# uc-vision/smart-tree

Hardware: AMD Instinct MI355X
Metric: points/sec end-to-end (voxelize->sparse-UNet->skeleton), 1M-pt tree (higher is better)
Workload: dtype f32

## Files before the change

smart_tree_amd/csrc/knn.hip:

```cpp
#include "st_common.h"
#include "st_grid.h"

#define KNN_BLOCK 256

#define KNN_MEAN_MULT 0.45f

__global__ void k_grid_init(StGrid* g) {
    if (threadIdx.x == 0 && blockIdx.x == 0) {
        for (int a = 0; a < 3; a++) { g->lo_ord[a] = 0xffffffffu; g->hi_ord[a] = 0u; }
        g->rmax_ord = 0u;
        g->bound_sum_fix = 0ull;
        g->bound_cnt = 0ull;
        g->r = 0.0f;
    }
    if (blockIdx.x == 0 && threadIdx.x < ST_MAX_SEG) { g->seg_rmax_ord[threadIdx.x] = 0u; g->seg_r[threadIdx.x] = 0.0f; }
}

__device__ __forceinline__ unsigned grid_wave_min(unsigned v) { for (int d = 32; d > 0; d >>= 1) { const unsigned o = __shfl_xor(v, d); v = o < v ? o : v; } return v; }
__device__ __forceinline__ unsigned grid_wave_max(unsigned v) { for (int d = 32; d > 0; d >>= 1) { const unsigned o = __shfl_xor(v, d); v = o > v ? o : v; } return v; }

__global__ void __launch_bounds__(KNN_BLOCK) k_bound_max(const float* bound, int64_t n, StGrid* g, const int* seg_off, const uint8_t* valid) {
    __shared__ unsigned m;
    __shared__ unsigned long long sum, cnt;
    if (threadIdx.x == 0) { m = 0u; sum = 0ull; cnt = 0ull; }
    __syncthreads();
    const int seg = blockIdx.y;
    const int64_t i0 = seg_off ? seg_off[seg] : 0, i1 = seg_off ? seg_off[seg + 1] : n;
    unsigned mine = 0u;
    unsigned long long fix = 0ull;
    unsigned long long seen = 0ull;
    for (int64_t i = i0 + (int64_t)blockIdx.x * blockDim.x + threadIdx.x; i < i1; i += (int64_t)gridDim.x * blockDim.x) {
        if (valid && !valid[i]) continue;
        const float b = bound[i];
        if (b != b) continue;
        const unsigned o = st_f2ord(b);
        if (o > mine) mine = o;
        fix += (unsigned long long)(fminf(fmaxf(b, 0.0f), 128.0f) * 65536.0f);
        seen++;
    }
    mine = grid_wave_max(mine);
    for (int d = 32; d > 0; d >>= 1) { fix += __shfl_xor(fix, d); seen += __shfl_xor(seen, d); }
    if ((threadIdx.x & 63) == 0) { if (mine) atomicMax(&m, mine); atomicAdd(&sum, fix); atomicAdd(&cnt, seen); }
    __syncthreads();
    if (threadIdx.x == 0) {
        if (m) { atomicMax(&g->rmax_ord, m); atomicMax(&g->seg_rmax_ord[seg], m); }
        if (sum) atomicAdd(&g->bound_sum_fix, sum);
        if (cnt) atomicAdd(&g->bound_cnt, cnt);
    }
}

__global__ void __launch_bounds__(KNN_BLOCK) k_grid_bbox(const float* pts, int64_t n, StGrid* g, const uint8_t* valid) {
    __shared__ unsigned lo[3], hi[3];
    if (threadIdx.x < 3) { lo[threadIdx.x] = 0xffffffffu; hi[threadIdx.x] = 0u; }
    __syncthreads();
    unsigned l[3] = {0xffffffffu, 0xffffffffu, 0xffffffffu}, h[3] = {0u, 0u, 0u};
    const int64_t total = 3 * n, step = (int64_t)gridDim.x * blockDim.x;
    const int64_t e0 = (int64_t)blockIdx.x * blockDim.x + threadIdx.x;
    const int step3 = (int)(step % 3);
    int a = (int)(e0 % 3);
    for (int64_t e = e0; e < total; e += step, a = (a + step3) % 3) {
        const float pv = pts[e];
        if (valid && !valid[e / 3]) continue;
        if (!(fabsf(pv) <= 3.0e38f)) continue;
        const unsigned o = st_f2ord(pv);
#pragma unroll
        for (int k = 0; k < 3; k++)
            if (a == k) { l[k] = o < l[k] ? o : l[k]; h[k] = o > h[k] ? o : h[k]; }
    }
#pragma unroll
    for (int a = 0; a < 3; a++) { l[a] = grid_wave_min(l[a]); h[a] = grid_wave_max(h[a]); }
    if ((threadIdx.x & 63) == 0)
        for (int a = 0; a < 3; a++) { atomicMin(&lo[a], l[a]); atomicMax(&hi[a], h[a]); }
    __syncthreads();
    if (threadIdx.x < 3 && lo[threadIdx.x] <= hi[threadIdx.x]) {
        atomicMin(&g->lo_ord[threadIdx.x], lo[threadIdx.x]);
        atomicMax(&g->hi_ord[threadIdx.x], hi[threadIdx.x]);
    }
}

__global__ void k_grid_dims(StGrid* g, float cell, int64_t max_cells, float r, int nseg, float mean_mult, int64_t n_bound) {
    if (threadIdx.x != 0 || blockIdx.x != 0) return;
    float lo[3], hi[3];
    for (int a = 0; a < 3; a++) { lo[a] = st_ord2f(g->lo_ord[a]); hi[a] = st_ord2f(g->hi_ord[a]); g->lo[a] = lo[a]; }
    for (int s = 0; s < nseg; s++) g->seg_r[s] = r < 0.0f ? st_ord2f(g->seg_rmax_ord[s]) : r;
    if (r < 0.0f) r = st_ord2f(g->rmax_ord);
    g->r = r;
    if (cell < 0.0f) {
        cell = r / -cell;
        if (mean_mult > 0.0f && n_bound > 0 && g->bound_cnt > 0ull) {
            const float mean = (float)((double)g->bound_sum_fix / 65536.0 / (double)g->bound_cnt);
            if (mean > 0.0f) cell = fminf(cell, mean_mult * mean);
        }
        cell = fmaxf(cell, 1e-4f);
    }
    if (!(cell > 0.0f) || !(cell <= 3.0e38f)) cell = 1.0f;
    g->nseg = nseg;
    for (int a = 0; a < 3; a++)
        if (!(hi[a] >= lo[a])) { lo[a] = hi[a] = 0.0f; g->lo[a] = 0.0f; }
    for (int it = 0;; it++) {
        double total = (double)nseg;
        for (int a = 0; a < 3; a++) {
            float ext = (hi[a] - lo[a]) / cell;
            int d = ext < 2.0e9f ? (int)floorf(ext) + 1 : 0x7fffffff;
            if (d < 1 || it >= 300) d = 1;
            g->dim[a] = d;
            total *= (double)d;
        }
        if (total <= (double)max_cells) break;
        cell *= 2.0f;
    }
    g->seg_dim0 = g->dim[0];
    g->dim[0] = g->seg_dim0 * nseg;
    g->cell = cell;
    g->ncell = (int64_t)g->dim[0] * g->dim[1] * g->dim[2];
}

__global__ void k_grid_ncell1(const StGrid* g, int64_t* out) { *out = g->ncell + 1; }

__global__ void __launch_bounds__(KNN_BLOCK) k_grid_count(const float* pts, int64_t n, const StGrid* g, uint32_t* counts,
                                                          const int* seg_off, int nseg, uint32_t* pt_cell, uint32_t* pt_rank,
                                                          const uint8_t* valid) {
    for (int64_t i = (int64_t)blockIdx.x * blockDim.x + threadIdx.x; i < n; i += (int64_t)gridDim.x * blockDim.x) {
        if (valid && !valid[i]) { pt_cell[i] = 0xffffffffu; continue; }
        const float x = pts[3 * i], y = pts[3 * i + 1], z = pts[3 * i + 2];
        const bool finite = fabsf(x) <= 3.0e38f && fabsf(y) <= 3.0e38f && fabsf(z) <= 3.0e38f;
        const int64_t c = st_grid_cell(g, finite ? x : g->lo[0], finite ? y : g->lo[1], finite ? z : g->lo[2], st_seg_find(seg_off, nseg, i));
        pt_cell[i] = (uint32_t)c;
        pt_rank[i] = atomicAdd(&counts[c], 1u);
    }
}

__global__ void __launch_bounds__(KNN_BLOCK) k_grid_fill(const float* pts, int64_t n, const uint32_t* cell_start,
                                                         const uint32_t* pt_cell, const uint32_t* pt_rank, float4* recs) {
    for (int64_t i = (int64_t)blockIdx.x * blockDim.x + threadIdx.x; i < n; i += (int64_t)gridDim.x * blockDim.x) {
        if (pt_cell[i] == 0xffffffffu) continue;
        const uint32_t pos = cell_start[pt_cell[i]] + pt_rank[i];
        recs[pos] = make_float4(pts[3 * i], pts[3 * i + 1], pts[3 * i + 2], __uint_as_float((unsigned)i));
    }
}

int64_t st_grid_ws_bytes(int64_t n, int64_t max_cells) {
    StArena a(nullptr, 0);
    a.take<uint32_t>(n);
    a.take<uint32_t>(n);
    a.take<int64_t>(1);
    a.take<char>(st_scan_ws_bytes(max_cells + 1));
    return a.used;
}

int st_grid_build(const float* pts, int64_t n, float cell, int64_t max_cells, StGrid* g, uint32_t* cell_start, float4* recs,
                  void* ws, int64_t ws_bytes, hipStream_t stream, float r, const float* bound, int64_t n_bound,
                  const int* seg_off, int nseg, const int* bound_seg_off, float mean_mult, const uint8_t* valid) {
    if (nseg < 1 || nseg > ST_MAX_SEG) { st_set_error("grid: 1 <= clouds per batch <= %d (got %d)", ST_MAX_SEG, nseg); return ST_ERR_INVALID; }
    if (!seg_off) nseg = 1;
    StArena a(ws, ws_bytes);
    uint32_t* pt_cell = a.take<uint32_t>(n);
    uint32_t* pt_rank = a.take<uint32_t>(n);
    int64_t* ncell1_dev = a.take<int64_t>(1);
    int64_t scan_bytes = st_scan_ws_bytes(max_cells + 1);
    char* scan_ws = a.take<char>(scan_bytes);
    if (!pt_cell || !pt_rank || !ncell1_dev || !scan_ws) {
        st_set_error("grid: workspace too small (%lld < %lld)", (long long)ws_bytes, (long long)a.used);
        return ST_ERR_WORKSPACE;
    }
    unsigned gb = (unsigned)st_min64(st_div_up(n > 0 ? n : 1, KNN_BLOCK), 4096);
    hipLaunchKernelGGL(k_grid_init, dim3(1), dim3(64), 0, stream, g);
    static_assert(ST_MAX_SEG <= 64, "k_grid_init clears the per-cloud radii with one wavefront");
    hipLaunchKernelGGL(k_grid_bbox, dim3((unsigned)st_min64(st_div_up(3 * (n > 0 ? n : 1), (int64_t)KNN_BLOCK * 8), 512)), dim3(KNN_BLOCK), 0, stream, pts, n, g, valid);
    const int64_t ncell = st_min64(max_cells, 128 * n + 65536);
    if (r < 0.0f && bound && n_bound > 0)
        hipLaunchKernelGGL(k_bound_max, dim3((unsigned)st_min64(st_div_up(n_bound, (int64_t)KNN_BLOCK * nseg * 8), 512 / nseg + 1), (unsigned)nseg),
                           dim3(KNN_BLOCK), 0, stream, bound, n_bound, g, nseg > 1 ? (bound_seg_off ? bound_seg_off : seg_off) : (const int*)nullptr,
                           valid);
    hipLaunchKernelGGL(k_grid_dims, dim3(1), dim3(64), 0, stream, g, cell, ncell, r, nseg, mean_mult,
                       (r < 0.0f && bound) ? n_bound : (int64_t)0);
    if (getenv("ST_GRID_DEBUG")) {
        StGrid h;
        (void)hipMemcpyAsync(&h, g, sizeof(StGrid), hipMemcpyDeviceToHost, stream);
        st_stream_wait(stream);
        fprintf(stderr, "grid: n=%lld cell=%g ncell=%lld of %lld dims=%d,%d,%d\n", (long long)n, h.cell, (long long)h.ncell,
                (long long)ncell, h.dim[0], h.dim[1], h.dim[2]);
    }
    hipLaunchKernelGGL(k_grid_ncell1, dim3(1), dim3(1), 0, stream, (const StGrid*)g, ncell1_dev);
    st_fill_u32_dev(cell_start, ncell + 1, ncell1_dev, 0u, stream);
    hipLaunchKernelGGL(k_grid_count, dim3(gb), dim3(KNN_BLOCK), 0, stream, pts, n, (const StGrid*)g, cell_start, seg_off, nseg,
                       pt_cell, pt_rank, valid);
    ST_TRY(st_exclusive_scan_u32(cell_start, cell_start, ncell + 1, nullptr, scan_ws, scan_bytes, stream, ncell1_dev));
    hipLaunchKernelGGL(k_grid_fill, dim3(gb), dim3(KNN_BLOCK), 0, stream, pts, n, (const uint32_t*)cell_start,
                       (const uint32_t*)pt_cell, (const uint32_t*)pt_rank, recs);
    ST_CHECK_LAUNCH();
    return ST_OK;
}


#define KNN_WAVES (KNN_BLOCK / 64)
#define KNN_MASK_WORDS 64
#define KNN_CAP 128

__device__ __forceinline__ uint32_t knn_wave_scan(uint32_t v, int lane) {
    for (int d = 1; d < 64; d <<= 1) { const uint32_t o = __shfl_up(v, (unsigned)d); if (lane >= d) v += o; }
    return v;
}

__device__ __forceinline__ float knn_d2_max(float bound, bool strict) {
    if (!(bound >= 0.0f)) return -1.0f;
    if (bound == __uint_as_float(0x7f800000u)) return strict ? __uint_as_float(0x7f7fffffu) : bound;
    auto pass = [&](float x) { const float s = sqrtf(x); return strict ? s < bound : s <= bound; };
    unsigned b = __float_as_uint(bound * bound);
    if (b > 0x7f7fffffu) b = 0x7f7fffffu;
    while (!pass(__uint_as_float(b))) { if (b == 0u) return -1.0f; b--; }
    while (b < 0x7f7fffffu && pass(__uint_as_float(b + 1u))) b++;
    return __uint_as_float(b);
}

struct __attribute__((aligned(16))) KnnPair { unsigned long long x, y; };

template <int NCH, class F>
__device__ __forceinline__ void knn_rank(const unsigned long long* keys, int n, int lane, F emit) {
    unsigned long long mine[NCH];
    int rank[NCH];
#pragma unroll
    for (int c = 0; c < NCH; c++) {
        const int j = c * 64 + lane;
        mine[c] = j < n ? keys[j] : ~0ull;
        rank[c] = 0;
    }
    int t = 0;
    for (; t + 4 <= n; t += 4) {
        const KnnPair a = *reinterpret_cast<const KnnPair*>(keys + t), b = *reinterpret_cast<const KnnPair*>(keys + t + 2);
#pragma unroll
        for (int c = 0; c < NCH; c++)
            rank[c] += (a.x < mine[c] ? 1 : 0) + (a.y < mine[c] ? 1 : 0) + (b.x < mine[c] ? 1 : 0) + (b.y < mine[c] ? 1 : 0);
    }
    for (; t < n; t++) {
        const unsigned long long kt = keys[t];
#pragma unroll
        for (int c = 0; c < NCH; c++) rank[c] += kt < mine[c] ? 1 : 0;
    }
    __builtin_amdgcn_wave_barrier();
#pragma unroll
    for (int c = 0; c < NCH; c++)
        if (c * 64 + lane < n) emit(mine[c], rank[c]);
}

template <int K>
__device__ __forceinline__ int knn_cut(unsigned long long* keys, int n, int lane) {
    __builtin_amdgcn_wave_barrier();
    auto put = [&](unsigned long long key, int rank) { if (rank < K) keys[rank] = key; };
    if (n <= 64) knn_rank<1>(keys, n, lane, put); else knn_rank<KNN_CAP / 64>(keys, n, lane, put);
    __builtin_amdgcn_wave_barrier();
    return n < K ? n : K;
}

template <int K, bool COUNT = false>
__global__ void __launch_bounds__(KNN_BLOCK, 8) k_knn(const float* __restrict__ src, int64_t n1, const StGrid* __restrict__ g,
                                                   const uint32_t* __restrict__ cell_start, const float4* __restrict__ recs,
                                                   float r, const float* __restrict__ bound, int mode,
                                                   int64_t* __restrict__ idx_out, float* __restrict__ dist_out,
                                                   const int* __restrict__ seg_off, int nseg, int cell_order,
                                                   const uint8_t* __restrict__ valid = nullptr) {
    __shared__ uint32_t s_roff[KNN_WAVES][65], s_rfirst[KNN_WAVES][64];
    __shared__ unsigned long long s_rmask[KNN_WAVES][KNN_MASK_WORDS];
    __shared__ __attribute__((aligned(16))) unsigned long long s_keys[KNN_WAVES][KNN_CAP];
    const int lane = threadIdx.x & 63, wave = threadIdx.x >> 6;
    int64_t i = (int64_t)blockIdx.x * KNN_WAVES + wave;
    if (i >= n1) return;
    if (valid && (cell_order ? i >= (int64_t)cell_start[g->ncell] : !valid[i])) return;
    float px, py, pz;
    if (cell_order) {
        const float4 me = recs[i];
        px = me.x; py = me.y; pz = me.z;
        i = (int64_t)__float_as_uint(me.w);
    } else {
        px = src[3 * i]; py = src[3 * i + 1]; pz = src[3 * i + 2];
    }
    uint32_t* roff = s_roff[wave];
    uint32_t* rfirst = s_rfirst[wave];
    unsigned long long* rmask = s_rmask[wave];
    unsigned long long* keys = s_keys[wave];
    const int seg = st_seg_find(seg_off, nseg, i);
    if (r < 0.0f) r = g->seg_r[seg];
    const float r2 = r * r;
    float reach_r = r;
    float d2_max = __uint_as_float(0x7f800000u);
    if (mode != 0) {
        const float bnd = bound[i];
        if (bnd < reach_r) reach_r = bnd;
        d2_max = knn_d2_max(bnd, mode == 2);
    }
    const float cell = g->cell;
    const float reach_f = reach_r > 0.0f ? ceilf(reach_r / cell) : 0.0f;
    int reach = reach_f < 1.0e6f ? (int)reach_f : 1000000;
    if (reach < 1) reach = 1;
    const bool q_finite = fabsf(px) <= 3.0e38f && fabsf(py) <= 3.0e38f && fabsf(pz) <= 3.0e38f;
    if (!q_finite) { px = g->lo[0]; py = g->lo[1]; pz = g->lo[2]; reach = 0; d2_max = -1.0f; }
    const int cx = (int)floorf((px - g->lo[0]) / cell), cy = (int)floorf((py - g->lo[1]) / cell), cz = (int)floorf((pz - g->lo[2]) / cell);
    const int xoff = seg * g->seg_dim0;
    const int x0 = st_max(cx - reach, 0), x1 = st_min(cx + reach, g->seg_dim0 - 1);
    const int y0 = st_max(cy - reach, 0), y1 = st_min(cy + reach, g->dim[1] - 1);
    const int z0 = st_max(cz - reach, 0), z1 = st_min(cz + reach, g->dim[2] - 1);
    const float rs = reach_r * 1.0001f + 1e-7f, rs2 = rs * rs;
    const int ny = y1 - y0 + 1, nrows = (x1 >= x0 && ny > 0 && z1 >= z0) ? (x1 - x0 + 1) * ny : 0;
    int nkeys = 0;
    unsigned long long thr = ~0ull;
    for (int rbase = 0; rbase < nrows && !(COUNT && nkeys >= K); rbase += 64) {
        const int rowi = rbase + lane;
        uint32_t first = 0, cnt = 0;
        if (rowi < nrows) {
            const int x = x0 + rowi / ny, y = y0 + rowi % ny;
            const float cx0 = g->lo[0] + (float)x * cell, ex = px < cx0 ? cx0 - px : (px > cx0 + cell ? px - (cx0 + cell) : 0.0f);
            const float cy0 = g->lo[1] + (float)y * cell, ey = py < cy0 ? cy0 - py : (py > cy0 + cell ? py - (cy0 + cell) : 0.0f);
            const float dxy2 = ex * ex + ey * ey;
            if (!(dxy2 > rs2)) {
                const float rz = sqrtf(rs2 - dxy2);
                const int za = (int)fmaxf(floorf((pz - rz - g->lo[2]) / cell) - 1.0f, (float)z0),
                          zb = (int)fminf(floorf((pz + rz - g->lo[2]) / cell) + 1.0f, (float)z1);
                if (za <= zb) {
                    const int64_t row = ((int64_t)(xoff + x) * g->dim[1] + y) * g->dim[2];
                    first = cell_start[row + za];
                    cnt = cell_start[row + zb + 1] - first;
                }
            }
        }
        const uint32_t incl = knn_wave_scan(cnt, lane);
        const int total = (int)__shfl(incl, 63);
        const unsigned long long nonempty = __ballot(cnt != 0u);
        const int nr = __popcll(nonempty);
        const int slot = __popcll(nonempty & ((1ull << lane) - 1ull));
        const bool marks = total <= 64 * KNN_MASK_WORDS;
        __builtin_amdgcn_wave_barrier();
        if (marks)
            for (int w = lane; w < (total + 63) / 64; w += 64) rmask[w] = 0ull;
        if (cnt != 0u) { roff[slot] = incl - cnt; rfirst[slot] = first; }
        if (lane == 63) roff[nr] = incl;
        __builtin_amdgcn_wave_barrier();
        if (marks && cnt != 0u) atomicOr(&rmask[(incl - cnt) >> 6], 1ull << ((incl - cnt) & 63u));
        __builtin_amdgcn_wave_barrier();
        int rows_before = 0;
        for (int cb = 0; cb < total && !(COUNT && nkeys >= K); cb += 64) {
            const int t = cb + lane;
            bool ok = false;
            unsigned long long key = 0ull;
            const unsigned long long starts = marks ? rmask[cb >> 6] : 0ull;
            if (t < total) {
                int lo;
                if (marks) {
                    lo = rows_before + __popcll(starts & (~0ull >> (63 - lane))) - 1;
                } else {
                    lo = 0;
                    int hi = nr;
                    while (hi - lo > 1) { const int mid = (lo + hi) >> 1; if (roff[mid] <= (uint32_t)t) lo = mid; else hi = mid; }
                }
                const float4 q = recs[rfirst[lo] + ((uint32_t)t - roff[lo])];
                const float dx = px - q.x, dy = py - q.y, dz = pz - q.z;
                float d2 = dx * dx;
                float tt = dy * dy;
                d2 = d2 + tt;
                tt = dz * dz;
                d2 = d2 + tt;
                ok = d2 < r2 && d2 <= d2_max;
                key = ((unsigned long long)__float_as_uint(d2) << 32) | (unsigned long long)__float_as_uint(q.w);
                if (!COUNT) ok = ok && key < thr;
            }
            const unsigned long long bal = __ballot(ok);
            if (!COUNT && ok) keys[nkeys + __popcll(bal & ((1ull << lane) - 1ull))] = key;
            nkeys += __popcll(bal);
            if (!COUNT && nkeys > KNN_CAP - 64) {
                nkeys = knn_cut<K>(keys, nkeys, lane);
                if (nkeys == K) thr = keys[K - 1];
            }
            rows_before += __popcll(starts);
        }
    }
    if (COUNT) {
        if (lane == 0) reinterpret_cast<uint8_t*>(idx_out)[i] = nkeys >= K ? 1 : 0;
        return;
    }
    __builtin_amdgcn_wave_barrier();
    {
        auto put = [&](unsigned long long key, int rank) {
            if (rank < K) {
                idx_out[i * K + rank] = (int64_t)(unsigned)(key & 0xffffffffull);
                dist_out[i * K + rank] = sqrtf(__uint_as_float((unsigned)(key >> 32)));
            }
        };
        if (nkeys <= 64) knn_rank<1>(keys, nkeys, lane, put); else knn_rank<KNN_CAP / 64>(keys, nkeys, lane, put);
        const int found = nkeys < K ? nkeys : K;
        if (lane >= found && lane < K) {
            idx_out[i * K + lane] = (int64_t)-1;
            dist_out[i * K + lane] = __uint_as_float(0x7fc00000u);
        }
    }
}

#define KNN_MAX_CELLS (1ll << 24)
static inline int64_t knn_max_cells(int nseg) { return KNN_MAX_CELLS * (nseg < 1 ? 1 : (nseg > 32 ? 32 : nseg)); }

static inline int64_t knn_cells(int64_t n2, int nseg) { return st_min64(knn_max_cells(nseg), 128 * (n2 > 0 ? n2 : 1) + 65536); }

static void knn_layout(StArena& a, int64_t n2, int nseg, StGrid** g, uint32_t** cell_start, float4** recs, char** sub, int64_t* sub_bytes) {
    *g = a.take<StGrid>(1);
    *cell_start = a.take<uint32_t>(knn_cells(n2, nseg) + 1);
    *recs = a.take<float4>(n2);
    *sub_bytes = st_grid_ws_bytes(n2, knn_cells(n2, nseg));
    *sub = a.take<char>(*sub_bytes);
}

extern "C" int64_t st_knn_workspace_bytes_seg(int64_t n_dst, int nseg) {
    StArena a(nullptr, 0);
    StGrid* g; uint32_t* cs; float4* recs; char* sub; int64_t sb;
    knn_layout(a, n_dst, nseg, &g, &cs, &recs, &sub, &sb);
    return a.used;
}
extern "C" int64_t st_knn_workspace_bytes(int64_t n_dst) { return st_knn_workspace_bytes_seg(n_dst, 1); }

extern "C" int st_knn_radius_seg(const float* src, int64_t n1, const float* dst, int64_t n2, int K, float r, const float* bound,
                                 int bound_mode, float cell_hint, int64_t* idx, float* dist, const int32_t* src_seg_off,
                                 const int32_t* dst_seg_off, int nseg, void* ws, int64_t ws_bytes, void* stream_,
                                 float cell_mean_mult) {
    hipStream_t stream = (hipStream_t)stream_;
    ST_REQUIRE(K == 1 || K == 8 || K == 16 || K == 32 || K == 64, "knn: K must be 1, 8, 16, 32 or 64 (got %d)", K);
    static_assert(KNN_CAP >= 128, "a cut keeps K <= 64 keys and the next chunk adds up to 64");
    ST_REQUIRE(bound_mode == 0 || bound != nullptr, "knn: bound_mode needs a bound array");
    ST_REQUIRE(r >= 0.0f || bound != nullptr, "knn: r < 0 (radius = max(bound)) needs a bound array");
    ST_REQUIRE(cell_hint >= 0.0f || r < 0.0f, "knn: a relative cell size (cell_hint < 0) goes with r < 0");
    ST_REQUIRE(n2 < (1ll << 31), "knn: too many points");
    ST_REQUIRE(nseg >= 1 && nseg <= ST_MAX_SEG, "knn: 1 <= clouds per batch <= %d", ST_MAX_SEG);
    ST_REQUIRE(nseg == 1 || (src_seg_off && dst_seg_off), "knn: a batch needs the cloud offsets of src and dst");
    if (nseg == 1) { src_seg_off = nullptr; dst_seg_off = nullptr; }
    if (n1 <= 0) return ST_OK;
    StArena a(ws, ws_bytes);
    StGrid* g; uint32_t* cell_start; float4* recs; char* sub; int64_t sub_bytes;
    knn_layout(a, n2, nseg, &g, &cell_start, &recs, &sub, &sub_bytes);
    if (!a.ok() || !sub) {
        st_set_error("knn: workspace too small (%lld < %lld)", (long long)ws_bytes, (long long)a.used);
        return ST_ERR_WORKSPACE;
    }
    const float cell_arg = cell_hint != 0.0f ? cell_hint : (r >= 0.0f ? r : -1.0f);
    ST_TRY(st_grid_build(dst, n2, cell_arg, knn_cells(n2, nseg), g, cell_start, recs, sub, sub_bytes, stream, r, bound, n1,
                         dst_seg_off, nseg, src_seg_off, cell_hint < 0.0f ? (cell_mean_mult >= 0.0f ? cell_mean_mult : KNN_MEAN_MULT) : 0.0f, nullptr));
    dim3 grid((unsigned)st_div_up(n1, KNN_WAVES)), block(KNN_BLOCK);
    const int cell_order = src == dst && n1 == n2 ? 1 : 0;
    if (K == 1)
        hipLaunchKernelGGL((k_knn<1>), grid, block, 0, stream, src, n1, (const StGrid*)g, (const uint32_t*)cell_start,
                           (const float4*)recs, r, bound, bound_mode, idx, dist, src_seg_off, nseg, cell_order);
    else if (K == 8)
        hipLaunchKernelGGL((k_knn<8>), grid, block, 0, stream, src, n1, (const StGrid*)g, (const uint32_t*)cell_start,
                           (const float4*)recs, r, bound, bound_mode, idx, dist, src_seg_off, nseg, cell_order);
    else if (K == 16)
        hipLaunchKernelGGL((k_knn<16>), grid, block, 0, stream, src, n1, (const StGrid*)g, (const uint32_t*)cell_start,
                           (const float4*)recs, r, bound, bound_mode, idx, dist, src_seg_off, nseg, cell_order);
    else if (K == 32)
        hipLaunchKernelGGL((k_knn<32>), grid, block, 0, stream, src, n1, (const StGrid*)g, (const uint32_t*)cell_start,
                           (const float4*)recs, r, bound, bound_mode, idx, dist, src_seg_off, nseg, cell_order);
    else
        hipLaunchKernelGGL((k_knn<64>), grid, block, 0, stream, src, n1, (const StGrid*)g, (const uint32_t*)cell_start,
                           (const float4*)recs, r, bound, bound_mode, idx, dist, src_seg_off, nseg, cell_order);
    ST_CHECK_LAUNCH();
    return ST_OK;
}

extern "C" int st_radius_count_seg(const float* src, int64_t n1, const float* dst, int64_t n2, int K, float r, const float* bound,
                                   int bound_mode, float cell_hint, uint8_t* mask, const int32_t* src_seg_off,
                                   const int32_t* dst_seg_off, int nseg, void* ws, int64_t ws_bytes, void* stream_,
                                   float cell_mean_mult, const uint8_t* valid) {
    hipStream_t stream = (hipStream_t)stream_;
    ST_REQUIRE(valid == nullptr || (src == dst && n1 == n2), "radius_count: a validity mask needs src == dst");
    ST_REQUIRE(K == 8, "radius_count: K must be 8 (outlier_removal's nb_points; got %d)", K);
    ST_REQUIRE(bound_mode == 0 || bound != nullptr, "radius_count: bound_mode needs a bound array");
    ST_REQUIRE(r >= 0.0f || bound != nullptr, "radius_count: r < 0 (radius = max(bound)) needs a bound array");
    ST_REQUIRE(cell_hint >= 0.0f || r < 0.0f, "radius_count: a relative cell size (cell_hint < 0) goes with r < 0");
    ST_REQUIRE(n2 < (1ll << 31), "radius_count: too many points");
    ST_REQUIRE(nseg >= 1 && nseg <= ST_MAX_SEG, "radius_count: 1 <= clouds per batch <= %d", ST_MAX_SEG);
    ST_REQUIRE(nseg == 1 || (src_seg_off && dst_seg_off), "radius_count: a batch needs the cloud offsets of src and dst");
    if (nseg == 1) { src_seg_off = nullptr; dst_seg_off = nullptr; }
    if (n1 <= 0) return ST_OK;
    StArena a(ws, ws_bytes);
    StGrid* g; uint32_t* cell_start; float4* recs; char* sub; int64_t sub_bytes;
    knn_layout(a, n2, nseg, &g, &cell_start, &recs, &sub, &sub_bytes);
    if (!a.ok() || !sub) {
        st_set_error("radius_count: workspace too small (%lld < %lld)", (long long)ws_bytes, (long long)a.used);
        return ST_ERR_WORKSPACE;
    }
    const float cell_arg = cell_hint != 0.0f ? cell_hint : (r >= 0.0f ? r : -1.0f);
    ST_TRY(st_grid_build(dst, n2, cell_arg, knn_cells(n2, nseg), g, cell_start, recs, sub, sub_bytes, stream, r, bound, n1,
                         dst_seg_off, nseg, src_seg_off, cell_hint < 0.0f ? (cell_mean_mult >= 0.0f ? cell_mean_mult : KNN_MEAN_MULT) : 0.0f, valid));
    if (valid) (void)hipMemsetAsync(mask, 0, (size_t)n1, stream);
    hipLaunchKernelGGL((k_knn<8, true>), dim3((unsigned)st_div_up(n1, KNN_WAVES)), dim3(KNN_BLOCK), 0, stream, src, n1,
                       (const StGrid*)g, (const uint32_t*)cell_start, (const float4*)recs, r, bound, bound_mode,
                       reinterpret_cast<int64_t*>(mask), (float*)nullptr, src_seg_off, nseg, src == dst && n1 == n2 ? 1 : 0, valid);
    ST_CHECK_LAUNCH();
    return ST_OK;
}

extern "C" int st_knn_radius(const float* src, int64_t n1, const float* dst, int64_t n2, int K, float r, const float* bound,
                             int bound_mode, float cell_hint, int64_t* idx, float* dist, void* ws, int64_t ws_bytes,
                             void* stream_) {
    return st_knn_radius_seg(src, n1, dst, n2, K, r, bound, bound_mode, cell_hint, idx, dist, nullptr, nullptr, 1, ws, ws_bytes,
                             stream_, -1.0f);
}
```

smart_tree_amd/csrc/prims.hip:

```cpp
#include <cstdarg>

#include "st_common.h"

static thread_local char g_err[512] = "";

void st_set_error(const char* fmt, ...) {
    va_list ap;
    va_start(ap, fmt);
    vsnprintf(g_err, sizeof(g_err), fmt, ap);
    va_end(ap);
}

extern "C" const char* st_last_error(void) { return g_err; }
void st_stream_wait(hipStream_t stream) { (void)hipStreamSynchronize(stream); }

extern "C" int st_version(void) { return 115; }

#define SCAN_BLOCK 256
#define SCAN_ITEMS 16
#define SCAN_TILE (SCAN_BLOCK * SCAN_ITEMS)
#define SCAN_DIRECT_BLOCKS 1024

__device__ __forceinline__ void scan_load(const uint32_t* in, int64_t base, int64_t n, uint32_t (&v)[SCAN_ITEMS]) {
    if (base + SCAN_ITEMS <= n && ((((uintptr_t)in) & 15) == 0)) {
        const uint4* p = reinterpret_cast<const uint4*>(in + base);
#pragma unroll
        for (int q = 0; q < SCAN_ITEMS / 4; q++) {
            const uint4 t = p[q];
            v[4 * q] = t.x; v[4 * q + 1] = t.y; v[4 * q + 2] = t.z; v[4 * q + 3] = t.w;
        }
    } else {
#pragma unroll
        for (int i = 0; i < SCAN_ITEMS; i++) v[i] = base + i < n ? in[base + i] : 0u;
    }
}

__global__ void __launch_bounds__(SCAN_BLOCK) k_scan_reduce(const uint32_t* in, uint32_t* block_sums, int64_t n, const int64_t* n_dev) {
    __shared__ uint32_t lds[SCAN_BLOCK / 64 + 1];
    if (n_dev) {
        const int64_t m = *n_dev;
        n = m < n ? m : n;
        if ((int64_t)blockIdx.x * SCAN_TILE >= n) { if (threadIdx.x == 0) block_sums[blockIdx.x] = 0u; return; }
    }
    int64_t base = (int64_t)blockIdx.x * SCAN_TILE + (int64_t)threadIdx.x * SCAN_ITEMS;
    uint32_t v[SCAN_ITEMS];
    scan_load(in, base, n, v);
    uint32_t s = 0;
#pragma unroll
    for (int i = 0; i < SCAN_ITEMS; i++) s += v[i];
    uint32_t total;
    block_exclusive_scan(s, lds, &total);
    if (threadIdx.x == 0) block_sums[blockIdx.x] = total;
}

__global__ void __launch_bounds__(SCAN_BLOCK) k_scan_apply(const uint32_t* in, uint32_t* out, const uint32_t* block_sums,
                                                           int64_t n, uint32_t* total_out, int sums_scanned, const int64_t* n_dev) {
    __shared__ uint32_t lds[SCAN_BLOCK / 64 + 1];
    if (n_dev) {
        const int64_t m = *n_dev;
        n = m < n ? m : n;
        const bool last_live = (int64_t)blockIdx.x * SCAN_TILE < n && ((int64_t)blockIdx.x + 1) * SCAN_TILE >= n;
        if ((int64_t)blockIdx.x * SCAN_TILE >= n && !(n == 0 && blockIdx.x == 0)) return;
        if (total_out && !last_live && !(n == 0)) total_out = nullptr;
    } else if (blockIdx.x != gridDim.x - 1) {
        total_out = nullptr;
    }
    uint32_t carry;
    if (sums_scanned) {
        carry = block_sums[blockIdx.x];
    } else {
        uint32_t pre = 0;
        for (int64_t j = threadIdx.x; j < (int64_t)blockIdx.x; j += SCAN_BLOCK) pre += block_sums[j];
        block_exclusive_scan(pre, lds, &carry);
    }
    int64_t base = (int64_t)blockIdx.x * SCAN_TILE + (int64_t)threadIdx.x * SCAN_ITEMS;
    uint32_t v[SCAN_ITEMS];
    scan_load(in, base, n, v);
    uint32_t s = 0;
#pragma unroll
    for (int i = 0; i < SCAN_ITEMS; i++) s += v[i];
    uint32_t total;
    uint32_t ex = block_exclusive_scan(s, lds, &total) + carry;
    if (base + SCAN_ITEMS <= n && ((((uintptr_t)out) & 15) == 0)) {
        uint4* p = reinterpret_cast<uint4*>(out + base);
#pragma unroll
        for (int q = 0; q < SCAN_ITEMS / 4; q++) {
            uint4 t;
            t.x = ex; ex += v[4 * q];
            t.y = ex; ex += v[4 * q + 1];
            t.z = ex; ex += v[4 * q + 2];
            t.w = ex; ex += v[4 * q + 3];
            p[q] = t;
        }
    } else {
#pragma unroll
        for (int i = 0; i < SCAN_ITEMS; i++) {
            if (base + i < n) out[base + i] = ex;
            ex += v[i];
        }
    }
    if (total_out && threadIdx.x == 0) *total_out = carry + total;
}

int64_t st_scan_ws_bytes(int64_t n) {
    StArena a(nullptr, 0);
    for (int64_t nb = st_div_up(n > 0 ? n : 1, SCAN_TILE);; nb = st_div_up(nb, SCAN_TILE)) {
        a.take<uint32_t>(nb + 1);
        if (nb <= SCAN_DIRECT_BLOCKS) break;
    }
    return a.used;
}

static int scan_level(const uint32_t* in, uint32_t* out, int64_t n, uint32_t* total, StArena& a, hipStream_t stream,
                      const int64_t* n_dev = nullptr) {
    const int64_t nb = st_div_up(n, SCAN_TILE);
    uint32_t* sums = a.take<uint32_t>(nb + 1);
    if (!sums) {
        st_set_error("scan: workspace too small (%lld < %lld)", (long long)a.size, (long long)a.used);
        return ST_ERR_WORKSPACE;
    }
    hipLaunchKernelGGL(k_scan_reduce, dim3((unsigned)nb), dim3(SCAN_BLOCK), 0, stream, in, sums, n, n_dev);
    const bool deep = nb > SCAN_DIRECT_BLOCKS;
    if (deep) ST_TRY(scan_level(sums, sums, nb, sums + nb, a, stream));
    hipLaunchKernelGGL(k_scan_apply, dim3((unsigned)nb), dim3(SCAN_BLOCK), 0, stream, in, out, (const uint32_t*)sums, n, total,
                       deep ? 1 : 0, n_dev);
    return ST_OK;
}

int st_exclusive_scan_u32(const uint32_t* in, uint32_t* out, int64_t n, uint32_t* total, void* ws, int64_t ws_bytes,
                          hipStream_t stream, const int64_t* n_dev) {
    if (n <= 0) {
        if (total) (void)hipMemsetAsync(total, 0, sizeof(uint32_t), stream);
        return ST_OK;
    }
    StArena a(ws, ws_bytes);
    ST_TRY(scan_level(in, out, n, total, a, stream, n_dev));
    ST_CHECK_LAUNCH();
    return ST_OK;
}

__global__ void __launch_bounds__(SCAN_BLOCK) k_fill_u32_dev(uint32_t* p, int64_t n, const int64_t* n_dev, uint32_t value) {
    const int64_t m = *n_dev < n ? *n_dev : n;
    for (int64_t i = ((int64_t)blockIdx.x * blockDim.x + threadIdx.x) * 4; i < m; i += (int64_t)gridDim.x * blockDim.x * 4) {
        if (i + 4 <= m && ((((uintptr_t)p) & 15) == 0)) *reinterpret_cast<uint4*>(p + i) = make_uint4(value, value, value, value);
        else for (int64_t j = i; j < m && j < i + 4; j++) p[j] = value;
    }
}
void st_fill_u32_dev(uint32_t* p, int64_t n, const int64_t* n_dev, uint32_t value, hipStream_t stream) {
    if (n <= 0) return;
    const int64_t g = st_div_up(st_div_up(n, 4), SCAN_BLOCK);
    hipLaunchKernelGGL(k_fill_u32_dev, dim3((unsigned)(g < 16384 ? g : 16384)), dim3(SCAN_BLOCK), 0, stream, p, n, n_dev, value);
}

#define SORT_BLOCK 256
#define SORT_ITEMS 4
#define SORT_TILE (SORT_BLOCK * SORT_ITEMS)
#define SORT_WAVES (SORT_BLOCK / 64)

__global__ void __launch_bounds__(SORT_BLOCK) k_sort_hist(const uint32_t* keys, int64_t n, int shift, uint32_t* hist,
                                                          int64_t nb) {
    __shared__ uint32_t h[256];
    h[threadIdx.x] = 0;
    __syncthreads();
    int64_t base = (int64_t)blockIdx.x * SORT_TILE;
    for (int r = 0; r < SORT_ITEMS; r++) {
        int64_t e = base + (int64_t)r * SORT_BLOCK + threadIdx.x;
        if (e < n) atomicAdd(&h[(keys[e] >> shift) & 255u], 1u);
    }
    __syncthreads();
    hist[(int64_t)threadIdx.x * nb + blockIdx.x] = h[threadIdx.x];
}

__global__ void __launch_bounds__(SORT_BLOCK) k_sort_scatter(const uint32_t* keys, const uint32_t* vals, uint32_t* okeys,
                                                             uint32_t* ovals, int64_t n, int shift, const uint32_t* hist,
                                                             int64_t nb) {
    __shared__ uint32_t running[256];
    __shared__ uint32_t wd[SORT_WAVES][256];
    const int tid = threadIdx.x, lane = tid & 63, wave = tid >> 6;
    running[tid] = hist[(int64_t)tid * nb + blockIdx.x];
    for (int w = 0; w < SORT_WAVES; w++) wd[w][tid] = 0;
    __syncthreads();
    int64_t base = (int64_t)blockIdx.x * SORT_TILE;
    for (int r = 0; r < SORT_ITEMS; r++) {
        int64_t e = base + (int64_t)r * SORT_BLOCK + tid;
        bool valid = e < n;
        uint32_t key = valid ? keys[e] : 0u;
        uint32_t val = valid ? vals[e] : 0u;
        uint32_t digit = (key >> shift) & 255u;
        unsigned long long peers = __ballot(valid);
        for (int b = 0; b < 8; b++) {
            bool bit = (digit >> b) & 1u;
            unsigned long long bal = __ballot(valid && bit);
            peers &= bit ? bal : ~bal;
        }
        unsigned long long below = peers & ((1ull << lane) - 1ull);
        uint32_t rank = (uint32_t)__popcll(below);
        if (valid && rank == 0) wd[wave][digit] = (uint32_t)__popcll(peers);
        __syncthreads();
        if (valid) {
            uint32_t off = running[digit] + rank;
            for (int w = 0; w < wave; w++) off += wd[w][digit];
            okeys[off] = key;
            ovals[off] = val;
        }
        __syncthreads();
        uint32_t add = 0;
        for (int w = 0; w < SORT_WAVES; w++) {
            add += wd[w][tid];
            wd[w][tid] = 0;
        }
        running[tid] += add;
        __syncthreads();
    }
}

int64_t st_sort_ws_bytes(int64_t n) {
    if (n <= 0) n = 1;
    StArena a(nullptr, 0);
    int64_t nb = st_div_up(n, SORT_TILE);
    a.take<uint32_t>(n);
    a.take<uint32_t>(n);
    a.take<uint32_t>(256 * nb);
    a.take<char>(st_scan_ws_bytes(256 * nb));
    return a.used;
}

int st_radix_sort_pairs_u32(uint32_t* keys, uint32_t* vals, int64_t n, int key_bits, void* ws, int64_t ws_bytes,
                            hipStream_t stream) {
    if (n <= 1 || key_bits <= 0) return ST_OK;
    StArena a(ws, ws_bytes);
    int64_t nb = st_div_up(n, SORT_TILE);
    uint32_t* tk = a.take<uint32_t>(n);
    uint32_t* tv = a.take<uint32_t>(n);
    uint32_t* hist = a.take<uint32_t>(256 * nb);
    int64_t scan_bytes = st_scan_ws_bytes(256 * nb);
    char* scan_ws = a.take<char>(scan_bytes);
    if (!tk || !tv || !hist || !scan_ws) {
        st_set_error("sort: workspace too small (%lld < %lld)", (long long)ws_bytes, (long long)a.used);
        return ST_ERR_WORKSPACE;
    }
    uint32_t *ik = keys, *iv = vals, *ok = tk, *ov = tv;
    for (int shift = 0; shift < key_bits; shift += 8) {
        hipLaunchKernelGGL(k_sort_hist, dim3((unsigned)nb), dim3(SORT_BLOCK), 0, stream, (const uint32_t*)ik, n, shift,
                           hist, nb);
        ST_TRY(st_exclusive_scan_u32(hist, hist, 256 * nb, nullptr, scan_ws, scan_bytes, stream));
        hipLaunchKernelGGL(k_sort_scatter, dim3((unsigned)nb), dim3(SORT_BLOCK), 0, stream, (const uint32_t*)ik,
                           (const uint32_t*)iv, ok, ov, n, shift, (const uint32_t*)hist, nb);
        uint32_t* t;
        t = ik; ik = ok; ok = t;
        t = iv; iv = ov; ov = t;
    }
    if (ik != keys) {
        (void)hipMemcpyAsync(keys, ik, n * sizeof(uint32_t), hipMemcpyDeviceToDevice, stream);
        (void)hipMemcpyAsync(vals, iv, n * sizeof(uint32_t), hipMemcpyDeviceToDevice, stream);
    }
    ST_CHECK_LAUNCH();
    return ST_OK;
}

extern "C" int64_t st_scan_workspace_bytes(int64_t n) { return st_scan_ws_bytes(n); }
extern "C" int st_scan_u32(const uint32_t* in, uint32_t* out, int64_t n, uint32_t* total, void* ws, int64_t ws_bytes,
                           void* stream) {
    return st_exclusive_scan_u32(in, out, n, total, ws, ws_bytes, (hipStream_t)stream);
}
extern "C" int64_t st_sort_workspace_bytes(int64_t n) { return st_sort_ws_bytes(n); }
extern "C" int st_sort_pairs_u32(uint32_t* keys, uint32_t* vals, int64_t n, int key_bits, void* ws, int64_t ws_bytes,
                                 void* stream) {
    return st_radix_sort_pairs_u32(keys, vals, n, key_bits, ws, ws_bytes, (hipStream_t)stream);
}

extern "C" int64_t st_voxelize_workspace_bytes(int64_t, int, int64_t);
extern "C" int64_t st_strided_workspace_bytes(int64_t);
extern "C" int64_t st_knn_workspace_bytes(int64_t);
extern "C" int64_t st_make_edges_workspace_bytes(int64_t);
extern "C" int64_t st_component_layout_workspace_bytes(int64_t);
extern "C" int64_t st_component_csr_workspace_bytes(int64_t);
extern "C" int64_t st_skeleton_workspace_bytes(int64_t, int64_t);
extern "C" int64_t st_query_workspace(int op, int64_t a, int64_t b, int64_t c) {
    switch (op) {
        case 0: return st_scan_ws_bytes(a);
        case 1: return st_sort_ws_bytes(a);
        case 2: return st_voxelize_workspace_bytes(a, (int)b, c);
        case 3: return st_strided_workspace_bytes(a);
        case 4: return st_knn_workspace_bytes(a);
        case 5: return st_make_edges_workspace_bytes(a);
        case 6: return st_component_layout_workspace_bytes(a);
        case 7: return st_component_csr_workspace_bytes(a);
        case 8: return st_skeleton_workspace_bytes(a, b);
        default: st_set_error("st_query_workspace: unknown op %d", op); return -1;
    }
}
```

Baseline: 975.2 million.

## Process several queries per wave in kNN with prefetched row fetch; fold ncell1 kernel

The kNN kernel now assigns KNN_QW queries to each wavefront instead of one. Per-query setup is computed in parallel by the first lanes and staged in shared memory. The cell-range fetch for the next row batch, or for the next query, is issued before the current batch is processed, so global loads overlap the scan and distance work. Row and column indices now come from a reciprocal-multiply division instead of integer div/mod. Separately, the tiny ncell+1 kernel is merged into k_grid_dims to save one launch. The cost is fewer waves in flight and serial processing of queries within a wave, which can hurt latency hiding and load balance.

```diff
diff --git a/smart_tree_amd/csrc/knn.hip b/smart_tree_amd/csrc/knn.hip
--- a/smart_tree_amd/csrc/knn.hip
+++ b/smart_tree_amd/csrc/knn.hip
@@ -78,7 +78,8 @@
     }
 }
 
-__global__ void k_grid_dims(StGrid* g, float cell, int64_t max_cells, float r, int nseg, float mean_mult, int64_t n_bound) {
+__global__ void k_grid_dims(StGrid* g, float cell, int64_t max_cells, float r, int nseg, float mean_mult, int64_t n_bound,
+                            int64_t* ncell1_out) {
     if (threadIdx.x != 0 || blockIdx.x != 0) return;
     float lo[3], hi[3];
     for (int a = 0; a < 3; a++) { lo[a] = st_ord2f(g->lo_ord[a]); hi[a] = st_ord2f(g->hi_ord[a]); g->lo[a] = lo[a]; }
@@ -113,9 +114,9 @@
     g->dim[0] = g->seg_dim0 * nseg;
     g->cell = cell;
     g->ncell = (int64_t)g->dim[0] * g->dim[1] * g->dim[2];
-}
-
-__global__ void k_grid_ncell1(const StGrid* g, int64_t* out) { *out = g->ncell + 1; }
+    *ncell1_out = g->ncell + 1;
+}
+
 
 __global__ void __launch_bounds__(KNN_BLOCK) k_grid_count(const float* pts, int64_t n, const StGrid* g, uint32_t* counts,
                                                           const int* seg_off, int nseg, uint32_t* pt_cell, uint32_t* pt_rank,
@@ -173,7 +174,7 @@
                            dim3(KNN_BLOCK), 0, stream, bound, n_bound, g, nseg > 1 ? (bound_seg_off ? bound_seg_off : seg_off) : (const int*)nullptr,
                            valid);
     hipLaunchKernelGGL(k_grid_dims, dim3(1), dim3(64), 0, stream, g, cell, ncell, r, nseg, mean_mult,
-                       (r < 0.0f && bound) ? n_bound : (int64_t)0);
+                       (r < 0.0f && bound) ? n_bound : (int64_t)0, ncell1_dev);
     if (getenv("ST_GRID_DEBUG")) {
         StGrid h;
         (void)hipMemcpyAsync(&h, g, sizeof(StGrid), hipMemcpyDeviceToHost, stream);
@@ -181,7 +182,6 @@
         fprintf(stderr, "grid: n=%lld cell=%g ncell=%lld of %lld dims=%d,%d,%d\n", (long long)n, h.cell, (long long)h.ncell,
                 (long long)ncell, h.dim[0], h.dim[1], h.dim[2]);
     }
-    hipLaunchKernelGGL(k_grid_ncell1, dim3(1), dim3(1), 0, stream, (const StGrid*)g, ncell1_dev);
     st_fill_u32_dev(cell_start, ncell + 1, ncell1_dev, 0u, stream);
     hipLaunchKernelGGL(k_grid_count, dim3(gb), dim3(KNN_BLOCK), 0, stream, pts, n, (const StGrid*)g, cell_start, seg_off, nseg,
                        pt_cell, pt_rank, valid);
@@ -250,6 +250,35 @@
     if (n <= 64) knn_rank<1>(keys, n, lane, put); else knn_rank<KNN_CAP / 64>(keys, n, lane, put);
     __builtin_amdgcn_wave_barrier();
     return n < K ? n : K;
+}
+
+#ifndef KNN_QW
+#define KNN_QW 8
+#endif
+static_assert(KNN_QW >= 1 && KNN_QW <= 64, "one lane per query of the run resolves it");
+
+struct __attribute__((aligned(16))) KnnQ {
+    float px, py, pz, r2, d2_max, rs2;
+    int x0, y0, ny, nym, nrows, z0, z1, xoff;
+    unsigned i;
+    int act;
+};
+
+__device__ __forceinline__ float knn_uni_f(float v) { return __int_as_float(__builtin_amdgcn_readfirstlane(__float_as_int(v))); }
+__device__ __forceinline__ int knn_uni_i(int v) { return __builtin_amdgcn_readfirstlane(v); }
+__device__ __forceinline__ KnnQ knn_uni(const KnnQ& v) {
+    KnnQ Q;
+    Q.px = knn_uni_f(v.px); Q.py = knn_uni_f(v.py); Q.pz = knn_uni_f(v.pz);
+    Q.r2 = knn_uni_f(v.r2); Q.d2_max = knn_uni_f(v.d2_max); Q.rs2 = knn_uni_f(v.rs2);
+    Q.x0 = knn_uni_i(v.x0); Q.y0 = knn_uni_i(v.y0); Q.ny = knn_uni_i(v.ny); Q.nym = knn_uni_i(v.nym);
+    Q.nrows = knn_uni_i(v.nrows); Q.z0 = knn_uni_i(v.z0); Q.z1 = knn_uni_i(v.z1); Q.xoff = knn_uni_i(v.xoff);
+    Q.i = (unsigned)knn_uni_i((int)v.i);
+    Q.act = knn_uni_i(v.act);
+    return Q;
+}
+
+__device__ __forceinline__ int knn_rows_div(int t, int ny, int nym) {
+    return ny >= 64 ? (t >= ny ? 1 : 0) : (int)(((unsigned)t * (unsigned)nym) >> 16);
 }
 
 template <int K, bool COUNT = false>
@@ -262,133 +291,178 @@
     __shared__ uint32_t s_roff[KNN_WAVES][65], s_rfirst[KNN_WAVES][64];
     __shared__ unsigned long long s_rmask[KNN_WAVES][KNN_MASK_WORDS];
     __shared__ __attribute__((aligned(16))) unsigned long long s_keys[KNN_WAVES][KNN_CAP];
+    __shared__ KnnQ s_head[KNN_WAVES][KNN_QW];
     const int lane = threadIdx.x & 63, wave = threadIdx.x >> 6;
-    int64_t i = (int64_t)blockIdx.x * KNN_WAVES + wave;
-    if (i >= n1) return;
-    if (valid && (cell_order ? i >= (int64_t)cell_start[g->ncell] : !valid[i])) return;
-    float px, py, pz;
-    if (cell_order) {
-        const float4 me = recs[i];
-        px = me.x; py = me.y; pz = me.z;
-        i = (int64_t)__float_as_uint(me.w);
-    } else {
-        px = src[3 * i]; py = src[3 * i + 1]; pz = src[3 * i + 2];
+    const int64_t base = ((int64_t)blockIdx.x * KNN_WAVES + wave) * KNN_QW;
+    if (base >= n1) return;
+    int64_t nq = n1;
+    if (valid && cell_order) {
+        const int64_t in_table = (int64_t)cell_start[g->ncell];
+        if (in_table < nq) nq = in_table;
+        if (base >= nq) return;
     }
     uint32_t* roff = s_roff[wave];
     uint32_t* rfirst = s_rfirst[wave];
     unsigned long long* rmask = s_rmask[wave];
     unsigned long long* keys = s_keys[wave];
-    const int seg = st_seg_find(seg_off, nseg, i);
-    if (r < 0.0f) r = g->seg_r[seg];
-    const float r2 = r * r;
-    float reach_r = r;
-    float d2_max = __uint_as_float(0x7f800000u);
-    if (mode != 0) {
-        const float bnd = bound[i];
-        if (bnd < reach_r) reach_r = bnd;
-        d2_max = knn_d2_max(bnd, mode == 2);
-    }
-    const float cell = g->cell;
-    const float reach_f = reach_r > 0.0f ? ceilf(reach_r / cell) : 0.0f;
-    int reach = reach_f < 1.0e6f ? (int)reach_f : 1000000;
-    if (reach < 1) reach = 1;
-    const bool q_finite = fabsf(px) <= 3.0e38f && fabsf(py) <= 3.0e38f && fabsf(pz) <= 3.0e38f;
-    if (!q_finite) { px = g->lo[0]; py = g->lo[1]; pz = g->lo[2]; reach = 0; d2_max = -1.0f; }
-    const int cx = (int)floorf((px - g->lo[0]) / cell), cy = (int)floorf((py - g->lo[1]) / cell), cz = (int)floorf((pz - g->lo[2]) / cell);
-    const int xoff = seg * g->seg_dim0;
-    const int x0 = st_max(cx - reach, 0), x1 = st_min(cx + reach, g->seg_dim0 - 1);
-    const int y0 = st_max(cy - reach, 0), y1 = st_min(cy + reach, g->dim[1] - 1);
-    const int z0 = st_max(cz - reach, 0), z1 = st_min(cz + reach, g->dim[2] - 1);
-    const float rs = reach_r * 1.0001f + 1e-7f, rs2 = rs * rs;
-    const int ny = y1 - y0 + 1, nrows = (x1 >= x0 && ny > 0 && z1 >= z0) ? (x1 - x0 + 1) * ny : 0;
-    int nkeys = 0;
-    unsigned long long thr = ~0ull;
-    for (int rbase = 0; rbase < nrows && !(COUNT && nkeys >= K); rbase += 64) {
-        const int rowi = rbase + lane;
-        uint32_t first = 0, cnt = 0;
-        if (rowi < nrows) {
-            const int x = x0 + rowi / ny, y = y0 + rowi % ny;
-            const float cx0 = g->lo[0] + (float)x * cell, ex = px < cx0 ? cx0 - px : (px > cx0 + cell ? px - (cx0 + cell) : 0.0f);
-            const float cy0 = g->lo[1] + (float)y * cell, ey = py < cy0 ? cy0 - py : (py > cy0 + cell ? py - (cy0 + cell) : 0.0f);
+    const float cell = g->cell, lo0 = g->lo[0], lo1 = g->lo[1], lo2 = g->lo[2];
+    const int seg_dim0 = g->seg_dim0, dim1 = g->dim[1], dim2 = g->dim[2];
+    KnnQ h;
+    h.px = h.py = h.pz = h.r2 = h.rs2 = 0.0f;
+    h.d2_max = -1.0f;
+    h.x0 = h.y0 = h.ny = h.nym = h.nrows = h.z0 = h.z1 = h.xoff = h.act = 0;
+    h.i = 0;
+    if (lane < KNN_QW && base + lane < nq && !(valid && !cell_order && !valid[base + lane])) {
+        int64_t i = base + lane;
+        float px, py, pz;
+        if (cell_order) {
+            const float4 me = recs[i];
+            px = me.x; py = me.y; pz = me.z;
+            i = (int64_t)__float_as_uint(me.w);
+        } else {
+            px = src[3 * i]; py = src[3 * i + 1]; pz = src[3 * i + 2];
+        }
+        const int seg = st_seg_find(seg_off, nseg, i);
+        const float rq = r < 0.0f ? g->seg_r[seg] : r;
+        float reach_r = rq;
+        float d2_max = __uint_as_float(0x7f800000u);
+        if (mode != 0) {
+            const float bnd = bound[i];
+            if (bnd < reach_r) reach_r = bnd;
+            d2_max = knn_d2_max(bnd, mode == 2);
+        }
+        const float reach_f = reach_r > 0.0f ? ceilf(reach_r / cell) : 0.0f;
+        int reach = reach_f < 1.0e6f ? (int)reach_f : 1000000;
+        if (reach < 1) reach = 1;
+        const bool q_finite = fabsf(px) <= 3.0e38f && fabsf(py) <= 3.0e38f && fabsf(pz) <= 3.0e38f;
+        if (!q_finite) { px = lo0; py = lo1; pz = lo2; reach = 0; d2_max = -1.0f; }
+        const int cx = (int)floorf((px - lo0) / cell), cy = (int)floorf((py - lo1) / cell), cz = (int)floorf((pz - lo2) / cell);
+        const int x0 = st_max(cx - reach, 0), x1 = st_min(cx + reach, seg_dim0 - 1);
+        const int y0 = st_max(cy - reach, 0), y1 = st_min(cy + reach, dim1 - 1);
+        const int z0 = st_max(cz - reach, 0), z1 = st_min(cz + reach, dim2 - 1);
+        const float rs = reach_r * 1.0001f + 1e-7f;
+        const int ny = y1 - y0 + 1;
+        h.px = px; h.py = py; h.pz = pz;
+        h.r2 = rq * rq; h.d2_max = d2_max; h.rs2 = rs * rs;
+        h.x0 = x0; h.y0 = y0; h.z0 = z0; h.z1 = z1; h.ny = ny;
+        h.nym = ny > 0 && ny < 64 ? 65536 / ny + 1 : 0;
+        h.nrows = (x1 >= x0 && ny > 0 && z1 >= z0 && !(d2_max < 0.0f)) ? (x1 - x0 + 1) * ny : 0;
+        h.xoff = seg * seg_dim0;
+        h.i = (unsigned)i;
+        h.act = 1;
+    }
+    const KnnQ* head = s_head[wave];
+    if (lane < KNN_QW) s_head[wave][lane] = h;
+    __builtin_amdgcn_wave_barrier();
+    auto fetch = [&](const KnnQ& F, int rbase, int xb, int yb, uint32_t& first, uint32_t& cnt) {
+        first = 0; cnt = 0;
+        if (rbase + lane < F.nrows) {
+            const int t = yb + lane, dq = knn_rows_div(t, F.ny, F.nym);
+            const int x = F.x0 + xb + dq, y = F.y0 + (t - dq * F.ny);
+            const float cx0 = lo0 + (float)x * cell, ex = F.px < cx0 ? cx0 - F.px : (F.px > cx0 + cell ? F.px - (cx0 + cell) : 0.0f);
+            const float cy0 = lo1 + (float)y * cell, ey = F.py < cy0 ? cy0 - F.py : (F.py > cy0 + cell ? F.py - (cy0 + cell) : 0.0f);
             const float dxy2 = ex * ex + ey * ey;
-            if (!(dxy2 > rs2)) {
-                const float rz = sqrtf(rs2 - dxy2);
-                const int za = (int)fmaxf(floorf((pz - rz - g->lo[2]) / cell) - 1.0f, (float)z0),
-                          zb = (int)fminf(floorf((pz + rz - g->lo[2]) / cell) + 1.0f, (float)z1);
+            if (!(dxy2 > F.rs2)) {
+                const float rz = sqrtf(F.rs2 - dxy2);
+                const int za = (int)fmaxf(floorf((F.pz - rz - lo2) / cell) - 1.0f, (float)F.z0),
+                          zb = (int)fminf(floorf((F.pz + rz - lo2) / cell) + 1.0f, (float)F.z1);
                 if (za <= zb) {
-                    const int64_t row = ((int64_t)(xoff + x) * g->dim[1] + y) * g->dim[2];
+                    const int64_t row = ((int64_t)(F.xoff + x) * dim1 + y) * dim2;
                     first = cell_start[row + za];
                     cnt = cell_start[row + zb + 1] - first;
                 }
             }
         }
-        const uint32_t incl = knn_wave_scan(cnt, lane);
-        const int total = (int)__shfl(incl, 63);
-        const unsigned long long nonempty = __ballot(cnt != 0u);
-        const int nr = __popcll(nonempty);
-        const int slot = __popcll(nonempty & ((1ull << lane) - 1ull));
-        const bool marks = total <= 64 * KNN_MASK_WORDS;
-        __builtin_amdgcn_wave_barrier();
-        if (marks)
-            for (int w = lane; w < (total + 63) / 64; w += 64) rmask[w] = 0ull;
-        if (cnt != 0u) { roff[slot] = incl - cnt; rfirst[slot] = first; }
-        if (lane == 63) roff[nr] = incl;
-        __builtin_amdgcn_wave_barrier();
-        if (marks && cnt != 0u) atomicOr(&rmask[(incl - cnt) >> 6], 1ull << ((incl - cnt) & 63u));
-        __builtin_amdgcn_wave_barrier();
-        int rows_before = 0;
-        for (int cb = 0; cb < total && !(COUNT && nkeys >= K); cb += 64) {
-            const int t = cb + lane;
-            bool ok = false;
-            unsigned long long key = 0ull;
-            const unsigned long long starts = marks ? rmask[cb >> 6] : 0ull;
-            if (t < total) {
-                int lo;
-                if (marks) {
-                    lo = rows_before + __popcll(starts & (~0ull >> (63 - lane))) - 1;
-                } else {
-                    lo = 0;
-                    int hi = nr;
-                    while (hi - lo > 1) { const int mid = (lo + hi) >> 1; if (roff[mid] <= (uint32_t)t) lo = mid; else hi = mid; }
+    };
+    uint32_t pf_first = 0, pf_cnt = 0;
+    bool pf_ready = false;
+    for (int q = 0; q < KNN_QW && base + q < nq; q++) {
+        const bool has_next = q + 1 < KNN_QW && base + q + 1 < nq;
+        const KnnQ Q = knn_uni(head[q]);
+        if (!pf_ready) fetch(Q, 0, 0, 0, pf_first, pf_cnt);
+        pf_ready = false;
+        const float px = Q.px, py = Q.py, pz = Q.pz, r2 = Q.r2, d2_max = Q.d2_max;
+        const int64_t i = cell_order ? (int64_t)Q.i : base + q;
+        int nkeys = 0;
+        unsigned long long thr = ~0ull;
+        int xb = 0, yb = 0;
+        for (int rbase = 0; rbase < Q.nrows && !(COUNT && nkeys >= K); rbase += 64) {
+            const uint32_t first = pf_first, cnt = pf_cnt;
+            {
+                const int t = yb + 64, dq = knn_rows_div(t, Q.ny, Q.nym);
+                xb += dq; yb = t - dq * Q.ny;
+                const bool more = rbase + 64 < Q.nrows;
+                pf_ready = !more && has_next;
+                if (more) fetch(Q, rbase + 64, xb, yb, pf_first, pf_cnt);
+                else if (has_next) fetch(head[q + 1], 0, 0, 0, pf_first, pf_cnt);
+            }
+            const uint32_t incl = knn_wave_scan(cnt, lane);
+            const int total = (int)__shfl(incl, 63);
+            const unsigned long long nonempty = __ballot(cnt != 0u);
+            const int nr = __popcll(nonempty);
+            const int slot = __popcll(nonempty & ((1ull << lane) - 1ull));
+            const bool marks = total <= 64 * KNN_MASK_WORDS;
+            __builtin_amdgcn_wave_barrier();
+            if (marks)
+                for (int w = lane; w < (total + 63) / 64; w += 64) rmask[w] = 0ull;
+            if (cnt != 0u) { roff[slot] = incl - cnt; rfirst[slot] = first; }
+            if (lane == 63) roff[nr] = incl;
+            __builtin_amdgcn_wave_barrier();
+            if (marks && cnt != 0u) atomicOr(&rmask[(incl - cnt) >> 6], 1ull << ((incl - cnt) & 63u));
+            __builtin_amdgcn_wave_barrier();
+            int rows_before = 0;
+            for (int cb = 0; cb < total && !(COUNT && nkeys >= K); cb += 64) {
+                const int t = cb + lane;
+                bool ok = false;
+                unsigned long long key = 0ull;
+                const unsigned long long starts = marks ? rmask[cb >> 6] : 0ull;
+                if (t < total) {
+                    int lo;
+                    if (marks) {
+                        lo = rows_before + __popcll(starts & (~0ull >> (63 - lane))) - 1;
+                    } else {
+                        lo = 0;
+                        int hi = nr;
+                        while (hi - lo > 1) { const int mid = (lo + hi) >> 1; if (roff[mid] <= (uint32_t)t) lo = mid; else hi = mid; }
+                    }
+                    const float4 q = recs[rfirst[lo] + ((uint32_t)t - roff[lo])];
+                    const float dx = px - q.x, dy = py - q.y, dz = pz - q.z;
+                    float d2 = dx * dx;
+                    float tt = dy * dy;
+                    d2 = d2 + tt;
+                    tt = dz * dz;
+                    d2 = d2 + tt;
+                    ok = d2 < r2 && d2 <= d2_max;
+                    key = ((unsigned long long)__float_as_uint(d2) << 32) | (unsigned long long)__float_as_uint(q.w);
+                    if (!COUNT) ok = ok && key < thr;
                 }
-                const float4 q = recs[rfirst[lo] + ((uint32_t)t - roff[lo])];
-                const float dx = px - q.x, dy = py - q.y, dz = pz - q.z;
-                float d2 = dx * dx;
-                float tt = dy * dy;
-                d2 = d2 + tt;
-                tt = dz * dz;
-                d2 = d2 + tt;
-                ok = d2 < r2 && d2 <= d2_max;
-                key = ((unsigned long long)__float_as_uint(d2) << 32) | (unsigned long long)__float_as_uint(q.w);
-                if (!COUNT) ok = ok && key < thr;
+                const unsigned long long bal = __ballot(ok);
+                if (!COUNT && ok) keys[nkeys + __popcll(bal & ((1ull << lane) - 1ull))] = key;
+                nkeys += __popcll(bal);
+                if (!COUNT && nkeys > KNN_CAP - 64) {
+                    nkeys = knn_cut<K>(keys, nkeys, lane);
+                    if (nkeys == K) thr = keys[K - 1];
+                }
+                rows_before += __popcll(starts);
             }
-            const unsigned long long bal = __ballot(ok);
-            if (!COUNT && ok) keys[nkeys + __popcll(bal & ((1ull << lane) - 1ull))] = key;
-            nkeys += __popcll(bal);
-            if (!COUNT && nkeys > KNN_CAP - 64) {
-                nkeys = knn_cut<K>(keys, nkeys, lane);
-                if (nkeys == K) thr = keys[K - 1];
+        }
+        if (COUNT) {
+            if (Q.act && lane == 0) reinterpret_cast<uint8_t*>(idx_out)[i] = nkeys >= K ? 1 : 0;
+        } else if (Q.act) {
+            __builtin_amdgcn_wave_barrier();
+            auto put = [&](unsigned long long key, int rank) {
+                if (rank < K) {
+                    idx_out[i * K + rank] = (int64_t)(unsigned)(key & 0xffffffffull);
+                    dist_out[i * K + rank] = sqrtf(__uint_as_float((unsigned)(key >> 32)));
+                }
+            };
+            if (nkeys <= 64) knn_rank<1>(keys, nkeys, lane, put); else knn_rank<KNN_CAP / 64>(keys, nkeys, lane, put);
+            const int found = nkeys < K ? nkeys : K;
+            if (lane >= found && lane < K) {
+                idx_out[i * K + lane] = (int64_t)-1;
+                dist_out[i * K + lane] = __uint_as_float(0x7fc00000u);
             }
-            rows_before += __popcll(starts);
-        }
-    }
-    if (COUNT) {
-        if (lane == 0) reinterpret_cast<uint8_t*>(idx_out)[i] = nkeys >= K ? 1 : 0;
-        return;
-    }
-    __builtin_amdgcn_wave_barrier();
-    {
-        auto put = [&](unsigned long long key, int rank) {
-            if (rank < K) {
-                idx_out[i * K + rank] = (int64_t)(unsigned)(key & 0xffffffffull);
-                dist_out[i * K + rank] = sqrtf(__uint_as_float((unsigned)(key >> 32)));
-            }
-        };
-        if (nkeys <= 64) knn_rank<1>(keys, nkeys, lane, put); else knn_rank<KNN_CAP / 64>(keys, nkeys, lane, put);
-        const int found = nkeys < K ? nkeys : K;
-        if (lane >= found && lane < K) {
-            idx_out[i * K + lane] = (int64_t)-1;
-            dist_out[i * K + lane] = __uint_as_float(0x7fc00000u);
+            __builtin_amdgcn_wave_barrier();
         }
     }
 }
@@ -439,7 +513,7 @@
     const float cell_arg = cell_hint != 0.0f ? cell_hint : (r >= 0.0f ? r : -1.0f);
     ST_TRY(st_grid_build(dst, n2, cell_arg, knn_cells(n2, nseg), g, cell_start, recs, sub, sub_bytes, stream, r, bound, n1,
                          dst_seg_off, nseg, src_seg_off, cell_hint < 0.0f ? (cell_mean_mult >= 0.0f ? cell_mean_mult : KNN_MEAN_MULT) : 0.0f, nullptr));
-    dim3 grid((unsigned)st_div_up(n1, KNN_WAVES)), block(KNN_BLOCK);
+    dim3 grid((unsigned)st_div_up(n1, (int64_t)KNN_WAVES * KNN_QW)), block(KNN_BLOCK);
     const int cell_order = src == dst && n1 == n2 ? 1 : 0;
     if (K == 1)
         hipLaunchKernelGGL((k_knn<1>), grid, block, 0, stream, src, n1, (const StGrid*)g, (const uint32_t*)cell_start,
@@ -486,7 +560,7 @@
     ST_TRY(st_grid_build(dst, n2, cell_arg, knn_cells(n2, nseg), g, cell_start, recs, sub, sub_bytes, stream, r, bound, n1,
                          dst_seg_off, nseg, src_seg_off, cell_hint < 0.0f ? (cell_mean_mult >= 0.0f ? cell_mean_mult : KNN_MEAN_MULT) : 0.0f, valid));
     if (valid) (void)hipMemsetAsync(mask, 0, (size_t)n1, stream);
-    hipLaunchKernelGGL((k_knn<8, true>), dim3((unsigned)st_div_up(n1, KNN_WAVES)), dim3(KNN_BLOCK), 0, stream, src, n1,
+    hipLaunchKernelGGL((k_knn<8, true>), dim3((unsigned)st_div_up(n1, (int64_t)KNN_WAVES * KNN_QW)), dim3(KNN_BLOCK), 0, stream, src, n1,
                        (const StGrid*)g, (const uint32_t*)cell_start, (const float4*)recs, r, bound, bound_mode,
                        reinterpret_cast<int64_t*>(mask), (float*)nullptr, src_seg_off, nseg, src == dst && n1 == n2 ? 1 : 0, valid);
     ST_CHECK_LAUNCH();
diff --git a/smart_tree_amd/csrc/prims.hip b/smart_tree_amd/csrc/prims.hip
--- a/smart_tree_amd/csrc/prims.hip
+++ b/smart_tree_amd/csrc/prims.hip
@@ -14,7 +14,7 @@
 extern "C" const char* st_last_error(void) { return g_err; }
 void st_stream_wait(hipStream_t stream) { (void)hipStreamSynchronize(stream); }
 
-extern "C" int st_version(void) { return 115; }
+extern "C" int st_version(void) { return 116; }
 
 #define SCAN_BLOCK 256
 #define SCAN_ITEMS 16
```

Result: faster. 1.010 billion (median of 6 runs) (+3.6%).
